# uc-vision/taichi_gaussian_rasterizer

Measured on AMD Instinct MI355X. Metric: Mpixels/s fwd+bwd @ 2048x2048, 1M Gaussians, higher is better.
Workload: dtype f32

## Files before the change

### taichi_gaussian_rasterizer_amd/csrc/frame.cpp

```cpp

#include <string.h>

#include "gs_common.h"

namespace {

int64_t a256(int64_t bytes) { return gs_align_up(bytes > 0 ? bytes : 1, 256); }

struct Dims {
  int64_t n, P, T;
  int C, F, col0, RS, tiles_x, tiles_y, local_h, D;
  bool want_vis;
};

int frame_dims(const GsFrame* f, Dims* d) {
  GS_REQUIRE(f != nullptr, GS_ERR_INVALID_ARGUMENT, "frame: descriptor is NULL");
  if (int rc = gs_check_cfg(&f->cfg)) return rc;
  GS_REQUIRE(f->n >= 0 && f->n < (int64_t(1) << 31), GS_ERR_INVALID_ARGUMENT, "frame: %lld gaussians", (long long)f->n);
  GS_REQUIRE(f->width > 0 && f->height > 0, GS_ERR_INVALID_ARGUMENT, "frame: image size %dx%d", f->width, f->height);
  GS_REQUIRE(f->sh_degree >= -1 && f->sh_degree <= 3, GS_ERR_UNSUPPORTED, "frame: SH degree %d", f->sh_degree);
  GS_REQUIRE(f->channels >= 1 && f->channels <= (f->sh_degree >= 0 ? GS_MAX_SH_CHANNELS : GS_MAX_FEATURES - 2),
             GS_ERR_UNSUPPORTED, "frame: %d feature channels", f->channels);
  const int ts = f->cfg.tile_size;
  GsShard sh;
// ... 23 lines not shown

template <typename T>
T* at(void* base, int64_t off) { return reinterpret_cast<T*>(static_cast<char*>(base) + off); }

struct StageTimer {
  void* const* events;
  int rc = GS_OK;
  void mark(int stage, int end, void* stream) {
    if (!events || !events[2 * stage + end]) return;
    if (hipEventRecord(static_cast<hipEvent_t>(events[2 * stage + end]), static_cast<hipStream_t>(stream)) != hipSuccess) {
      gs_set_error("frame: hipEventRecord of a stage timer failed");
      rc = GS_ERR_LAUNCH;
    }
  }
};

}

int gs_project_fwd_ex(int64_t n, const float* position, const float* log_scaling, const float* rotation,
                      const float* alpha_logit, const float* T_camera_world, const float* projection, int32_t width,
                      int32_t height, double near_plane, double far_plane, const GsRasterConfig* cfg, float* points,
                      float* depth, float* ndc_depth, int64_t* indexes, int32_t* slot_of, int32_t* num_visible,
                      float* depth_features, int32_t depth_features_stride, float* camera_pos, void* scratch,
                      int64_t scratch_bytes, float* zero_rows, int32_t zero_row_floats, const GsMapBinPlan* bin,
                      void* stream);

extern "C" int gs_frame_layout(const GsFrame* f, GsFrameLayout* out) {
  Dims d;
  if (int rc = frame_dims(f, &d)) return rc;
  GS_REQUIRE(out != nullptr, GS_ERR_INVALID_ARGUMENT, "gs_frame_layout: layout is NULL");
// ... 157 lines not shown
  if (lists) {
    int32_t* touched = at<int32_t>(workspace, L.touched);
    if ((rc = gs_map_touched_list(d.n, v_dev, d.T, stage, map_bytes, touched, counts + 1, indexes, d.n,
                                  f->exchange_world, at<int64_t>(workspace, L.owner_counts), f->exchange_rank,
                                  counts + 2, stream)))
      return rc;
    if (f->sh_degree >= 0) {
      tm.mark(GS_FWD_COLOURS, 0, stream);
      if ((rc = gs_sh_fwd_rows(d.n, touched, counts + 1, d.C, f->sh_degree, feature, position, indexes, cam_pos, colours,
                               d.F, stream)))
        return rc;
      tm.mark(GS_FWD_COLOURS, 1, stream);
    }
  }
  const int32_t tile_hint = f->max_tile_hint > 0 ? -f->max_tile_hint : 0;
  tm.mark(GS_FWD_MAP_FINISH, 0, stream);
  if ((rc = gs_map_finish(d.n, v_dev, f->k_capacity, tile_hint, points, ndc, f->width, f->height, cfg, f->use_depth16,
                          tile_ranges, o2p, nullptr, at<char>(scratch, L.s_pairs), shard, stage, map_bytes,
                          stream)))
    return rc;
  tm.mark(GS_FWD_MAP_FINISH, 1, stream);
  tm.mark(GS_FWD_RASTER, 0, stream);
  if ((rc = gs_raster_fwd_bg(d.n, d.F, points, feats, tile_ranges, o2p, f->k_capacity, f->width, f->height, &rcfg,
                             tile_order, counts + 7, image, alpha, vis, shard, background, d.col0, stream)))
    return rc;
  tm.mark(GS_FWD_RASTER, 1, stream);
  if (f->render_depth &&
      (rc = gs_depth_split_fwd(d.P, d.C, image, alpha, 1e-6f, at<float>(workspace, L.out_image),
                               at<float>(workspace, L.img_depth), at<float>(workspace, L.img_var), stream)))
    return rc;
  if (f->render_median_depth) {
    GsRasterConfig pick = f->cfg;
    pick.use_alpha_blending = 0;
    pick.saturate_threshold = 0.5f;
    pick.compute_visibility = 0;
    pick.compute_point_heuristic = 0;
    if ((rc = gs_raster_fwd(d.n, 1, points, depth, tile_ranges, o2p, f->k_capacity, f->width, f->height, &pick,
                            tile_order, counts + 7, at<float>(workspace, L.median),
                            at<float>(scratch, L.s_median_cover), nullptr, shard, stream)))
// ... 216 lines not shown
```

### taichi_gaussian_rasterizer_amd/csrc/gs_common.h

```cpp
#pragma once

#include <hip/hip_runtime.h>
#include <stdint.h>
#include <stdio.h>

#include "../../include/gsplat_hip.h"

#define GS_WAVE 64

void gs_set_error(const char* fmt, ...);

#define GS_REQUIRE(cond, status, ...)  \
  do {                                 \
    if (!(cond)) {                     \
      gs_set_error(__VA_ARGS__);       \
      return (status);                 \
    }                                  \
  } while (0)

#define GS_CHECK_LAUNCH(name)                                                   \
  do {                                                                          \
    hipError_t e_ = hipGetLastError();                                          \
    if (e_ != hipSuccess) {                                                     \
      gs_set_error("%s: launch failed: %s", name, hipGetErrorString(e_));       \
// ... 101 lines not shown
  const void* st_rows;
  const int* block_offsets;
  const int* block_counts;
  int num_blocks;
  float inv_far, ndc_denom;
  float* points; float* depth; float* ndc; int64_t* indexes; int* slot_of; int* num_visible;
  float* depth_feat; int depth_feat_stride;
  void* zero_rows; int zero_row_v4;
};
int gs_map_compact_bin(const GsMapBinPlan* plan, const GsCompactArgs* c, void* stream);
int gs_map_bin_counters(const GsMapBinPlan* plan, int64_t n, int32_t** words, int32_t* count);
int gs_map_prepare_ex(int64_t v, const int32_t* v_dev, const float* points, int32_t width, int32_t height,
                      const GsRasterConfig* cfg, int64_t k_capacity, int32_t* tile_ranges, int32_t* counts_out,
                      int32_t* counts_host, int32_t* tile_order, const GsRowShard* shard, void* scratch,
                      int64_t scratch_bytes, int binned, void* stream);
int gs_rows_add(int64_t v, int32_t row_floats, float* rows, const float* add_points, const float* add_depth,
                int32_t depth_col, void* stream);

#ifdef __HIPCC__

__device__ __forceinline__ int gs_xcd_remap(int block, int n) {
  const int chunk = (n + 7) >> 3;
  const int item = (block & 7) * chunk + (block >> 3);
  return ((block >> 3) < chunk && item < n) ? item : -1;
}

template <int CTRL, int ROW_MASK = 0xf, int BANK_MASK = 0xf>
__device__ __forceinline__ float gs_dpp_add(float x) {
  const int moved = __builtin_amdgcn_update_dpp(0, __float_as_int(x), CTRL, ROW_MASK, BANK_MASK, false);
  return x + __int_as_float(moved);
// ... 173 lines not shown
```

### taichi_gaussian_rasterizer_amd/csrc/mapper.hip

```cpp

#include "gs_common.h"
#include "../../include/gs_detmath.h"

namespace {

struct GridQuery {
  float ib00, ib01, ib10, ib11;
  float rel_min_x, rel_min_y;
  int min_tx, min_ty, span_x, span_y;
};

__device__ __forceinline__ GridQuery grid_query(const float* g, int Wp, int Hp, int tile_size, float alpha_thr) {
  GridQuery q;
  const float mx = g[0], my = g[1], ax = g[2], ay = g[3], sgx = g[4], sgy = g[5], alpha = g[6];
  if (!(alpha > alpha_thr)) {
    q.ib00 = q.ib01 = q.ib10 = q.ib11 = q.rel_min_x = q.rel_min_y = 0.f;
    q.min_tx = q.min_ty = q.span_x = q.span_y = 0;
    return q;
  }
  const float gscale = gs_det_sqrtf(2.0f * gs_det_logf(__fdiv_rn(alpha, alpha_thr)));
  const float sx = sgx * gscale, sy = sgy * gscale;
  const float a2x = -ay, a2y = ax;
  const float v1x = ax * sx, v1y = ay * sx, v2x = a2x * sy, v2y = a2y * sy;
  const float ex = gs_det_sqrtf(v1x * v1x + v2x * v2x), ey = gs_det_sqrtf(v1y * v1y + v2y * v2y);
// ... 47 lines not shown
  int depth16;
  GsShard sh;
};

__device__ __forceinline__ bool any_owned_row(const GsShard& sh, int lo, int hi) { return gs_shard_any_row(sh, lo, hi); }
__device__ __forceinline__ int local_tile(const MapArgs& a, int gx, int gy) {
  return gs_shard_local_row(a.sh, gy) * a.tiles_wide + gx;
}

__device__ __forceinline__ int64_t live_count(const MapArgs& a) {
  if (a.v_dev == nullptr) return a.v;
  const int64_t d = *a.v_dev;
  return d < a.v ? d : a.v;
}

__device__ __forceinline__ int wave_inclusive_scan(int x) {
  x += __builtin_amdgcn_update_dpp(0, x, 0x111, 0xf, 0xf, true);
  x += __builtin_amdgcn_update_dpp(0, x, 0x112, 0xf, 0xf, true);
  x += __builtin_amdgcn_update_dpp(0, x, 0x114, 0xf, 0xf, true);
  x += __builtin_amdgcn_update_dpp(0, x, 0x118, 0xf, 0xf, true);
  x += __builtin_amdgcn_update_dpp(0, x, 0x142, 0xa, 0xf, false);
  x += __builtin_amdgcn_update_dpp(0, x, 0x143, 0xc, 0xf, false);
  return x;
}

__device__ __forceinline__ int block_exclusive_scan(int x, int* s_wave, int& sum) {
  const int lane = threadIdx.x & 63, wv = threadIdx.x >> 6;
  const int inc = wave_inclusive_scan(x);
  if (lane == 63) s_wave[wv] = inc;
  __syncthreads();
  int before = 0;
  sum = 0;
#pragma unroll
  for (int w = 0; w < 16; ++w) {
    const int tot = s_wave[w];
    sum += tot;
    before += w < wv ? tot : 0;
  }
  __syncthreads();
// ... 523 lines not shown
    }
  }
  for (uint64_t todo = wide_lanes; todo != 0ull; todo &= todo - 1ull) {
    const int gi = __shfl(i, __ffsll(static_cast<unsigned long long>(todo)) - 1);
    const GridQuery w = grid_query(a.points + 7 * int64_t(gi), a.Wp, a.Hp, a.tile_size, a.thr);
    const uint64_t pair = (uint64_t(depth_key(a.depth[gi], a.depth16 != 0)) << 32) | uint64_t(uint32_t(gi));
    const int total = w.span_x * w.span_y;
    for (int k = lane; k < total; k += 64) {
      const int ty = k / w.span_x, tx = k - ty * w.span_x;
      if (gs_shard_owns(a.sh, ty + w.min_ty) && test_tile(w, tx, ty, a.tile_size))
        place(tx + w.min_tx, ty + w.min_ty, pair);
    }
  }
}

template <int THREADS>
__device__ __forceinline__ void bitonic_sort(uint64_t* data, int n, int t) {
  int np2 = 1;
  while (np2 < n) np2 <<= 1;
  for (int k = 2; k <= np2; k <<= 1) {
    for (int i = t; i < n; i += THREADS) {
      const int l = i ^ (k - 1);
      if (l > i && l < n) {
        const uint64_t x = data[i], y = data[l];
        if (x > y) { data[i] = y; data[l] = x; }
      }
    }
    __syncthreads();
    for (int j = k >> 2; j > 0; j >>= 1) {
      for (int i = t; i < n; i += THREADS) {
        const int l = i ^ j;
        if (l > i && l < n) {
          const uint64_t x = data[i], y = data[l];
          if (x > y) { data[i] = y; data[l] = x; }
        }
      }
      __syncthreads();
    }
  }
}

template <int THREADS, int CAP>
__device__ __forceinline__ uint64_t* lds_merge_sort(uint64_t* a, uint64_t* b, int n, int t) {
  const int np = (n + 255) & ~255;
  for (int i = n + t; i < np; i += THREADS) a[i] = 0xFFFFFFFF00000000ull | uint64_t(i);
  __syncthreads();
  const int lane = t & 63;
  for (int base = (t >> 6) * 256; base < np; base += (THREADS >> 6) * 256) {
    uint64_t* chunk = a + base;
    uint64_t mine[4];
    int rank[4];
#pragma unroll
    for (int q = 0; q < 4; ++q) { mine[q] = chunk[q * 64 + lane]; rank[q] = 0; }
    for (int j = 0; j < 64; ++j) {
#pragma unroll
// ... 96 lines not shown
      data = lds_merge_sort<THREADS, CAP>(s_a, s_b, n, t);
    } else {
      __syncthreads();
      bitonic_sort<THREADS>(stage, n, t);
      data = stage;
    }
    for (int i = t; i < n; i += THREADS) {
      const uint64_t kv = data[i];
      keys_out[lo + i] = K(uint32_t(kv >> 32) ^ bias);
      values_out[lo + i] = values[lo + int(uint32_t(kv))];
    }
    __syncthreads();
  }
}

template <int R>
__device__ __forceinline__ void rank_sort_rows(uint64_t* s_key, int n, int lane, int start, int tile, int* o2p,
                                               uint64_t* keys_out, int shift) {
  uint64_t mine[R];
  int rank[R];
#pragma unroll
  for (int q = 0; q < R; ++q) {
    mine[q] = s_key[q * 64 + lane];
    rank[q] = 0;
  }
  if (R == 1) {
    for (int j = 0; j < n; ++j) rank[0] += s_key[j] < mine[0] ? 1 : 0;
  } else {
    for (int j = 0; j < 64; ++j) {
#pragma unroll
      for (int q = 0; q < R; ++q) rank[q] += s_key[q * 64 + j] < mine[q] ? 1 : 0;
    }
#pragma unroll
    for (int q = 0; q < R; ++q) s_key[q * 64 + rank[q]] = mine[q];
    __syncthreads();
#pragma unroll
    for (int q = 0; q < R; ++q) {
#pragma unroll
      for (int p = 0; p < R; ++p) {
        if (p == q) continue;
        const uint64_t* row = s_key + p * 64;
        int pos = 0;
#pragma unroll
        for (int step = 32; step >= 1; step >>= 1) pos += row[pos + step - 1] < mine[q] ? step : 0;
        pos += row[pos] < mine[q] ? 1 : 0;
        rank[q] += pos;
      }
    }
  }
#pragma unroll
  for (int q = 0; q < R; ++q) {
    if ((mine[q] >> 32) != 0xFFFFFFFFull) {
      o2p[start + rank[q]] = int(uint32_t(mine[q]));
      if (keys_out) keys_out[start + rank[q]] = (mine[q] >> 32) | (uint64_t(uint32_t(tile)) << shift);
    }
  }
}

#ifndef GS_SORT_BINS
#define GS_SORT_BINS 1
#endif
constexpr int SORT_BINS = 256, BIN_LIMIT = 40;

template <int R>
__device__ __forceinline__ bool bucket_sort_rows(uint64_t* s_key, int* s_hist, int n, int lane, int start, int tile,
                                                 int* o2p, uint64_t* keys_out, int shift) {
  uint64_t mine[R];
  uint32_t mn = 0xFFFFFFFFu, mx = 0u;
#pragma unroll
  for (int q = 0; q < R; ++q) {
    mine[q] = s_key[q * 64 + lane];
    if (q * 64 + lane < n) {
      const uint32_t hi = uint32_t(mine[q] >> 32);
      mn = min(mn, hi);
      mx = max(mx, hi);
    }
  }
#pragma unroll
  for (int off = 32; off > 0; off >>= 1) {
    mn = min(mn, uint32_t(__shfl_xor(int(mn), off)));
    mx = max(mx, uint32_t(__shfl_xor(int(mx), off)));
  }
  const float scale = float(SORT_BINS) / (float(mx - mn) + 1.0f);
#pragma unroll
  for (int k = 0; k < SORT_BINS / 64; ++k) s_hist[k * 64 + lane] = 0;
  __syncthreads();
  int bin[R], arrival[R];
#pragma unroll
  for (int q = 0; q < R; ++q) {
    bin[q] = 0; arrival[q] = 0;
    if (q * 64 + lane < n) {
      bin[q] = min(SORT_BINS - 1, int(float(uint32_t(mine[q] >> 32) - mn) * scale));
      arrival[q] = atomicAdd(&s_hist[bin[q]], 1);
    }
  }
  __syncthreads();
  int c[SORT_BINS / 64], local = 0, fullest = 0;
#pragma unroll
  for (int k = 0; k < SORT_BINS / 64; ++k) {
    c[k] = s_hist[lane * (SORT_BINS / 64) + k];
    local += c[k];
    fullest = max(fullest, c[k]);
  }
#pragma unroll
  for (int off = 32; off > 0; off >>= 1) fullest = max(fullest, __shfl_xor(fullest, off));
  if (fullest > BIN_LIMIT) return false;
  int run = wave_inclusive_scan(local) - local;
  __syncthreads();
#pragma unroll
  for (int k = 0; k < SORT_BINS / 64; ++k) {
    s_hist[lane * (SORT_BINS / 64) + k] = run;
    run += c[k];
  }
  if (lane == 63) s_hist[SORT_BINS] = run;
  __syncthreads();
#pragma unroll
  for (int q = 0; q < R; ++q)
    if (q * 64 + lane < n) s_key[s_hist[bin[q]] + arrival[q]] = mine[q];
  __syncthreads();
#pragma unroll
  for (int q = 0; q < R; ++q) {
    if (q * 64 + lane >= n) continue;
    const int b0 = s_hist[bin[q]], b1 = s_hist[bin[q] + 1];
    int rank = b0;
    for (int j = b0; j < b1; ++j) rank += s_key[j] < mine[q] ? 1 : 0;
    o2p[start + rank] = int(uint32_t(mine[q]));
    if (keys_out) keys_out[start + rank] = (mine[q] >> 32) | (uint64_t(uint32_t(tile)) << shift);
  }
  return true;
}

template <int RMAX>
__global__ __launch_bounds__(64, 6) void tile_rank_sort_kernel(int num_tiles, const int2* tile_ranges,
                                                            uint64_t* pairs, int* o2p, uint64_t* keys_out,
                                                            int depth16, int skip_full) {
  __shared__ uint64_t s_key[64 * RMAX];
  __shared__ int s_hist[SORT_BINS + 1];
  const int tile = gs_xcd_remap(blockIdx.x, num_tiles);
  if (tile < 0) return;
  const int2 r = tile_ranges[tile];
  const int n = r.y - r.x;
  if (n <= 0) return;
  const int lane = threadIdx.x;
  const int shift = depth16 ? 16 : 32;
  if (n > 64 * RMAX) {
// ... 404 lines not shown
                       m.region_start, m.chunk_start, hist, m.qcache);
    GS_CHECK_LAUNCH("gs_map_prepare/count");
  }
  hipLaunchKernelGGL(map_scan_kernel, dim3(tile_order ? 2 : 1), dim3(1024), 0, s, num_tiles, hist,
                     reinterpret_cast<int2*>(tile_ranges), cursors, counts_out, k_capacity, tile_order, v_dev,
                     counts_host, v > 0 ? m.region_start + rg.num_regions : nullptr);
  GS_CHECK_LAUNCH("gs_map_prepare/scan");
  return GS_OK;
}

extern "C" int gs_map_finish(int64_t v, const int32_t* v_dev, int64_t k, int32_t max_tile_count, const float* points,
                             const float* depth, int32_t width, int32_t height, const GsRasterConfig* cfg,
                             int32_t use_depth16, const int32_t* tile_ranges, int32_t* overlap_to_point,
                             uint64_t* sorted_keys, void* pair_scratch, const GsRowShard* shard, void* scratch,
                             int64_t scratch_bytes, void* stream) {
  MapArgs a;
  if (int rc = fill_args(a, v, points, depth, width, height, cfg, use_depth16, shard)) return rc;
  a.v_dev = v_dev;
  if (k == 0 || v == 0) return GS_OK;
  const int num_tiles = a.tiles_wide * a.sh.local_rows;
  GS_REQUIRE(points && depth && tile_ranges && overlap_to_point && pair_scratch && scratch, GS_ERR_INVALID_ARGUMENT,
             "gs_map_finish: NULL buffer");
  GS_REQUIRE(scratch_bytes >= gs_map_scratch_bytes(v, num_tiles), GS_ERR_SCRATCH_TOO_SMALL,
             "gs_map_finish: scratch too small");
  hipStream_t s = static_cast<hipStream_t>(stream);
  const MapScratch m = carve(scratch, v, num_tiles);
  int* cursors = m.cursors;
  const RegionGrid rg = make_grid(a);
  uint64_t* pairs = static_cast<uint64_t*>(pair_scratch);
  hipLaunchKernelGGL(emit_binned_kernel, dim3(unsigned(gs_div_up(v, CHUNK)) + unsigned(rg.num_regions)), dim3(CHUNK),
                     size_t(rg.win) * rg.win * 8, s,
                     a, rg, m.order, m.region_start, m.chunk_start, cursors, pairs, m.qcache);
  GS_CHECK_LAUNCH("gs_map_finish/emit");
  const int grid = 8 * int(gs_div_up(num_tiles, 8));
  const int2* r = reinterpret_cast<const int2*>(tile_ranges);
  const bool exact = max_tile_count > 0;
  const int guess = exact ? max_tile_count : (max_tile_count < 0 ? -max_tile_count : 1024);
  const bool big_pass = guess > 512;
  const int skip_full = (exact || big_pass) ? 1 : 0;
  int covered;
  if (guess <= 256) {
    covered = 256;
    hipLaunchKernelGGL((tile_rank_sort_kernel<4>), dim3(grid), dim3(64), 0, s, num_tiles, r, pairs, overlap_to_point,
                       sorted_keys, use_depth16, skip_full);
  } else {
    covered = 512;
    hipLaunchKernelGGL((tile_rank_sort_kernel<8>), dim3(grid), dim3(64), 0, s, num_tiles, r, pairs, overlap_to_point,
                       sorted_keys, use_depth16, skip_full);
  }
  if (big_pass) {
    constexpr int SMALL = 1024, MID = 2048, CAP = 8192;
    const bool mid_pass = guess > SMALL, huge_pass = guess > MID;
// ... 133 lines not shown
```

### taichi_gaussian_rasterizer_amd/csrc/raster_fwd.hip

```cpp

#include "gs_common.h"
#include "raster_pdf.h"

namespace {

struct FwdArgs {
  const float* points;
  const float* features;
  const int2* ranges;
  const int* o2p;
  float* image;
  float* alpha;
  float* visibility;
  int W, H, F;
  int tiles_wide;
  int tile_size;
  int sub_x, sub_y;
  int num_items;
  int num_tiles;
  const int* heavy;
  int heavy_cap;
  const int* tile_order;
  float cmax, thr, inv_thr, sat_level;
  float cut;
  int blend, vis, aa;
  GsShard sh;
  const float* bg;
  int bg_off;
};

__device__ __forceinline__ void tile_origin(const FwdArgs& a, int tile, int& x0, int& y0, int& yout0) {
  const int lty = tile / a.tiles_wide;
  x0 = (tile - lty * a.tiles_wide) * a.tile_size;
  y0 = gs_shard_global_row(a.sh, lty) * a.tile_size;
  yout0 = lty * a.tile_size;
}

template <int NB, int FP, int MODE>
__device__ __forceinline__ void raster_fwd_body(const FwdArgs& a, int tile, int x0, int y0, int yout0,
                                                float4 (*s_geo)[(MODE == 2 ? 3 : 2) + (FP + 3) / 4], float* s_vis,
                                                int* s_idx) {
  constexpr int GEO_V4 = MODE == 2 ? 3 : 2, FEAT_V4 = (FP + 3) / 4;
  constexpr bool FULL = MODE == 2, VIS = MODE == 1 || MODE == 2, QUANT = MODE == 3;
  const bool blend = QUANT ? false : (FULL ? a.blend != 0 : true);
  const int lane = threadIdx.x;
  const int lx = lane & 7, ly = lane >> 3;
  float Xf[NB], Yf[NB], Tr[NB], acc[NB][FP];
  bool inb[NB], done[NB];
#pragma unroll
  for (int b = 0; b < NB; ++b) {
    const int X = x0 + (b & 1) * 8 + lx, Y = y0 + (b >> 1) * 8 + ly;
    inb[b] = X < a.W && Y < a.H;
    Xf[b] = FULL ? float(X) + 0.5f : float((b & 1) * 8 + lx) + 0.5f;
    Yf[b] = FULL ? float(Y) + 0.5f : float((b >> 1) * 8 + ly) + 0.5f;
    Tr[b] = inb[b] ? 1.0f : 0.0f;
    done[b] = false;
#pragma unroll
    for (int c = 0; c < FP; ++c) acc[b][c] = 0.0f;
  }

  const int2 range_v = a.ranges[tile];
  int2 range;
  range.x = __builtin_amdgcn_readfirstlane(range_v.x);
  range.y = __builtin_amdgcn_readfirstlane(range_v.y);
  const float k_exp = 0.84932180028801904f;

  for (int g0 = range.x; g0 < range.y; g0 += 64) {
    int live = 0;
    if (blend) {
#pragma unroll
      for (int b = 0; b < NB; ++b)
        if (__ballot(Tr[b] > a.cut) != 0ull) live |= 1 << b;
    } else {
#pragma unroll
      for (int b = 0; b < NB; ++b)
        if (__ballot(inb[b] && !done[b]) != 0ull) live |= 1 << b;
    }
    if (live == 0) break;
    const int cnt = __builtin_amdgcn_readfirstlane(min(64, range.y - g0));
    int staged_mask = 0;
    if (lane < cnt) {
      const int idx = a.o2p[g0 + lane];
      const float* p = a.points + int64_t(idx) * 7;
      const float mx = p[0], my = p[1], ax = p[2], ay = p[3], sx = p[4], sy = p[5], al = p[6];
      const float isx = gs_rcp_fast(sx), isy = gs_rcp_fast(sy);
      const float Ax = ax * isx * k_exp, Ay = ay * isx * k_exp;
      const float Bx = -ay * isy * k_exp, By = ax * isy * k_exp;
      int mask = 0;
      if (FULL && a.aa) {
        mask = gs_sub_block_mask_antialias<NB>(ax, ay, sx, sy, al, a.inv_thr, s_sig(0.5f, isx) - s_sig(-0.5f, isx),
                                               s_sig(0.5f, isy) - s_sig(-0.5f, isy), float(x0) + 0.5f - mx,
                                               float(y0) + 0.5f - my);
      } else if (al > a.thr) {
        mask = gs_sub_block_mask<NB>(Ax, Ay, Bx, By, __log2f(al * a.inv_thr), float(x0) + 0.5f - mx,
                                     float(y0) + 0.5f - my);
      }
      staged_mask = mask;
// ... 115 lines not shown
    const int X = x0 + (b & 1) * 8 + lx, Y = y0 + (b >> 1) * 8 + ly;
    const int64_t pix = int64_t(Y - y0 + yout0) * a.W + X;
    float* out = a.image + pix * a.F;
    if (a.bg != nullptr) {
#pragma unroll
      for (int c = 0; c < FP; ++c)
        if (c >= a.bg_off && c < a.F) acc[b][c] = __builtin_fmaf(Tr[b], a.bg[c - a.bg_off], acc[b][c]);
    }
#pragma unroll
    for (int c = 0; c < FP; ++c)
      if (c < a.F) out[c] = acc[b][c];
    a.alpha[pix] = blend ? 1.0f - Tr[b] : (Tr[b] < 1.0f ? 1.0f : 0.0f);
  }
}

template <int NB, int FP, int MODE>
__global__ __launch_bounds__(64) void raster_fwd_kernel(const FwdArgs a) {
  __shared__ float4 s_geo[64][(MODE == 2 ? 3 : 2) + (FP + 3) / 4];
  __shared__ float s_vis[(MODE == 1 || MODE == 2) ? 64 : 1];
  __shared__ int s_idx[(MODE == 1 || MODE == 2) ? 64 : 1];
  const int per_tile = a.sub_x * a.sub_y;
  constexpr int RW = NB == 1 ? 8 : 16, RH = NB == 4 ? 16 : 8;
  int tile, quad;
  if (a.tile_order) {
    const int b = blockIdx.x;
    const int heavy = (NB > 1 && a.heavy) ? min(*a.heavy, a.heavy_cap) : 0;
    if (NB > 1 && b < 4 * heavy) {
      tile = a.tile_order[b >> 2];
      int x0, y0, yout0;
      tile_origin(a, tile, x0, y0, yout0);
      x0 += (b & 1) * 8; y0 += ((b >> 1) & 1) * 8; yout0 += ((b >> 1) & 1) * 8;
      if (x0 < a.W && y0 < a.H) raster_fwd_body<1, FP, MODE>(a, tile, x0, y0, yout0, s_geo, s_vis, s_idx);
      return;
    }
    const int c = b - 4 * heavy, rank = heavy + c / per_tile;
    if (rank >= a.num_tiles) return;
    tile = a.tile_order[rank];
    quad = c % per_tile;
  } else {
    const int item = gs_xcd_remap(blockIdx.x, a.num_items);
    if (item < 0) return;
    tile = item / per_tile;
    quad = item - tile * per_tile;
  }
  int x0, y0, yout0;
  tile_origin(a, tile, x0, y0, yout0);
  x0 += (quad % a.sub_x) * RW; y0 += (quad / a.sub_x) * RH; yout0 += (quad / a.sub_x) * RH;
  if (x0 >= a.W || y0 >= a.H) return;
  raster_fwd_body<NB, FP, MODE>(a, tile, x0, y0, yout0, s_geo, s_vis, s_idx);
}

template <int NB, int MODE>
int launch_fp(const FwdArgs& a, hipStream_t s) {
  const int grid = 8 * int(gs_div_up(a.num_items + (a.heavy ? 4 * a.heavy_cap : 0), 8));
  if (MODE == 3 && a.F == 1) hipLaunchKernelGGL((raster_fwd_kernel<NB, 1, MODE>), dim3(grid), dim3(64), 0, s, a);
  else if (a.F <= 3) hipLaunchKernelGGL((raster_fwd_kernel<NB, 3, MODE>), dim3(grid), dim3(64), 0, s, a);
  else if (a.F <= 5) hipLaunchKernelGGL((raster_fwd_kernel<NB, 5, MODE>), dim3(grid), dim3(64), 0, s, a);
  else if (a.F <= 8) hipLaunchKernelGGL((raster_fwd_kernel<NB, 8, MODE>), dim3(grid), dim3(64), 0, s, a);
  else hipLaunchKernelGGL((raster_fwd_kernel<NB, 32, MODE>), dim3(grid), dim3(64), 0, s, a);
  GS_CHECK_LAUNCH("gs_raster_fwd");
  return GS_OK;
}

}

extern "C" int gs_raster_fwd_bg(int64_t v, int32_t num_features, const float* points, const float* features,
                                const int32_t* tile_ranges, const int32_t* overlap_to_point, int64_t k, int32_t width,
                                int32_t height, const GsRasterConfig* cfg, const int32_t* tile_order,
                                const int32_t* heavy_tiles, float* image, float* alpha, float* visibility,
                                const GsRowShard* shard, const float* background, int32_t background_offset,
                                void* stream) {
  if (int rc = gs_check_cfg(cfg)) return rc;
  if (int rc = gs_check_background("gs_raster_fwd", cfg->use_alpha_blending, background != nullptr, background_offset,
                                   num_features))
    return rc;
  GS_REQUIRE(width > 0 && height > 0, GS_ERR_INVALID_ARGUMENT, "gs_raster_fwd: image size %dx%d", width, height);
  GS_REQUIRE(num_features >= 1 && num_features <= GS_MAX_FEATURES, GS_ERR_UNSUPPORTED,
             "gs_raster_fwd: feature width %d not in [1,%d]", num_features, GS_MAX_FEATURES);
  GS_REQUIRE(image && alpha && tile_ranges, GS_ERR_INVALID_ARGUMENT, "gs_raster_fwd: NULL output or ranges");
  GS_REQUIRE(k == 0 || (points && features && overlap_to_point), GS_ERR_INVALID_ARGUMENT,
             "gs_raster_fwd: NULL input with %lld overlaps", (long long)k);
  const bool vis = cfg->compute_visibility || cfg->compute_point_heuristic;
  GS_REQUIRE(!vis || visibility || v == 0, GS_ERR_INVALID_ARGUMENT, "gs_raster_fwd: visibility buffer is NULL");
  const int ts = cfg->tile_size;
  FwdArgs a;
  a.points = points; a.features = features; a.ranges = reinterpret_cast<const int2*>(tile_ranges);
  a.o2p = overlap_to_point; a.image = image; a.alpha = alpha; a.visibility = visibility;
  a.W = width; a.H = height; a.F = num_features;
  a.tiles_wide = int(gs_div_up(width, ts));
  a.tile_size = ts;
  if (int rc = gs_make_shard(shard, int(gs_div_up(height, ts)), &a.sh)) return rc;
  const int num_tiles = a.tiles_wide * a.sh.local_rows;
  if (num_tiles == 0) return GS_OK;
  const int nb = gs_raster_sub_blocks(cfg, num_tiles, 0);
  a.sub_x = ts / (nb == 1 ? 8 : 16);
  a.sub_y = ts / (nb == 4 ? 16 : 8);
  a.num_items = num_tiles * a.sub_x * a.sub_y;
  a.tile_order = tile_order;
  a.num_tiles = num_tiles;
  a.heavy = (tile_order && ts == 16 && nb > 1) ? heavy_tiles : nullptr;
  a.heavy_cap = num_tiles / 4;
  if (cfg->tune_no_heavy_split) a.heavy = nullptr;
  a.cmax = cfg->clamp_max_alpha; a.thr = cfg->alpha_threshold; a.inv_thr = 1.0f / cfg->alpha_threshold;
  a.sat_level = 1.0f - cfg->saturate_threshold;
  a.cut = cfg->forward_cut > 2.98023223876953125e-08f ? cfg->forward_cut : 2.98023223876953125e-08f;
  a.blend = cfg->use_alpha_blending; a.vis = vis; a.aa = cfg->antialias;
  a.bg = background; a.bg_off = background ? background_offset : 0;
  hipStream_t s = static_cast<hipStream_t>(stream);
  const int mode = (!a.blend && !a.aa && !a.vis) ? 3 : (!a.blend || a.aa) ? 2 : a.vis ? 1 : 0;
// ... 19 lines not shown
```

### taichi_gaussian_rasterizer_amd/fused.py

```python
from __future__ import annotations

import ctypes
import weakref

import torch

from . import _native as nv
from .data_types import RasterConfig
from .spherical_harmonics import check_sh_degree

_K_HINT = {}
FRAME_CALLS = True
_PINNED = {}


def _pinned_counts(dev: torch.device) -> torch.Tensor:
    ring = _PINNED.get(dev.index)
    if ring is None:
        ring = _PINNED[dev.index] = dict(bufs=[torch.empty((8,), dtype=torch.int32).pin_memory() for _ in range(4)],
                                         at=0)
    ring["at"] = (ring["at"] + 1) % len(ring["bufs"])
    return ring["bufs"][ring["at"]]


# ... 381 lines not shown
    def backward(ctx, *grads):
        return _FrameRender.backward(ctx, *grads)[:5] + (None,) * (len(ctx.needs_input_grad) - 5)


def fused_supported(gaussians, camera_params, use_sh: bool, render_median_depth: bool) -> bool:
    f = gaussians.feature
    if gaussians.position.shape[0] == 0 or not f.is_cuda or f.dtype != torch.float32:
        return False
    if use_sh:
        return f.ndim == 3 and f.shape[1] <= 8
    return f.ndim == 2 and 1 <= f.shape[1] <= 30


def _capacity(hint):
    k_cap = -(-(int(hint[0] * 1.25) + 4096) // 65536) * 65536
    tile_hint = next((c for c in (256, 512, 1024, 2048) if hint[1] <= c), 4096)
    return k_cap, tile_hint


def render_fused(gaussians, camera_params, config: RasterConfig, render_depth: bool, use_depth16: bool,
                 shard=None, group=None, render_median_depth: bool = False, exchange: str = "dense",
                 grad_mode: str = "replicated", owned=None, owned_range=None, sparse_grad: bool = False,
                 background=None, differentiable_weight: bool = False):
    import weakref

    from .renderer import Rendering
    if shard is not None and (background is not None or differentiable_weight):
        raise NotImplementedError("render_fused: a sharded frame has neither a background nor a differentiable "
                                  "image_weight (parallel.render_gaussians_sharded does not take the arguments)")
    holder = {}
    args = (gaussians.position.contiguous(), gaussians.log_scaling.contiguous(), gaussians.rotation.contiguous(),
# ... 40 lines not shown
```

Baseline: 3977.

## Defer per-tile depth sort into the forward raster kernel behind env flag

Adds an optional path where the map-finish stage skips its per-tile sort and the forward raster kernel sorts each tile's key segment in LDS (bucket or rank sort), then reads gaussian indices from shared memory. The sorted order is still written to overlap_to_point for the backward pass. The path is gated by the GS_SORT_IN_RASTER environment variable, so it is off by default. Separately, it adds waves-per-EU occupancy hints to the raster kernel and a 384 tile-hint bucket in the Python capacity helper; both of those apply unconditionally.

```diff
diff --git a/taichi_gaussian_rasterizer_amd/csrc/frame.cpp b/taichi_gaussian_rasterizer_amd/csrc/frame.cpp
--- a/taichi_gaussian_rasterizer_amd/csrc/frame.cpp
+++ b/taichi_gaussian_rasterizer_amd/csrc/frame.cpp
@@ -1,4 +1,5 @@
 
+#include <stdlib.h>
 #include <string.h>
 
 #include "gs_common.h"
@@ -61,6 +62,14 @@
     }
   }
 };
+
+int sort_in_raster_enabled() {
+  static const int on = [] {
+    const char* e = getenv("GS_SORT_IN_RASTER");
+    return (e != nullptr && e[0] == '1' && e[1] == '\0') ? 1 : 0;
+  }();
+  return on;
+}
 
 }
 
@@ -248,15 +257,17 @@
     }
   }
   const int32_t tile_hint = f->max_tile_hint > 0 ? -f->max_tile_hint : 0;
+  int32_t sort_deferred = 0;
   tm.mark(GS_FWD_MAP_FINISH, 0, stream);
-  if ((rc = gs_map_finish(d.n, v_dev, f->k_capacity, tile_hint, points, ndc, f->width, f->height, cfg, f->use_depth16,
-                          tile_ranges, o2p, nullptr, at<char>(scratch, L.s_pairs), shard, stage, map_bytes,
-                          stream)))
+  if ((rc = gs_map_finish_ex(d.n, v_dev, f->k_capacity, tile_hint, points, ndc, f->width, f->height, cfg,
+                             f->use_depth16, tile_ranges, o2p, nullptr, at<char>(scratch, L.s_pairs), shard, stage,
+                             map_bytes, sort_in_raster_enabled(), &sort_deferred, stream)))
     return rc;
   tm.mark(GS_FWD_MAP_FINISH, 1, stream);
   tm.mark(GS_FWD_RASTER, 0, stream);
-  if ((rc = gs_raster_fwd_bg(d.n, d.F, points, feats, tile_ranges, o2p, f->k_capacity, f->width, f->height, &rcfg,
-                             tile_order, counts + 7, image, alpha, vis, shard, background, d.col0, stream)))
+  if ((rc = gs_raster_fwd_ex(d.n, d.F, points, feats, tile_ranges, o2p, f->k_capacity, f->width, f->height, &rcfg,
+                             tile_order, counts + 7, image, alpha, vis, shard, background, d.col0,
+                             sort_deferred ? at<uint64_t>(scratch, L.s_pairs) : nullptr, stream)))
     return rc;
   tm.mark(GS_FWD_RASTER, 1, stream);
   if (f->render_depth &&
diff --git a/taichi_gaussian_rasterizer_amd/csrc/gs_common.h b/taichi_gaussian_rasterizer_amd/csrc/gs_common.h
--- a/taichi_gaussian_rasterizer_amd/csrc/gs_common.h
+++ b/taichi_gaussian_rasterizer_amd/csrc/gs_common.h
@@ -139,6 +139,17 @@
                       const GsRasterConfig* cfg, int64_t k_capacity, int32_t* tile_ranges, int32_t* counts_out,
                       int32_t* counts_host, int32_t* tile_order, const GsRowShard* shard, void* scratch,
                       int64_t scratch_bytes, int binned, void* stream);
+#define GS_RASTER_SORT_MAX 384
+int gs_map_finish_ex(int64_t v, const int32_t* v_dev, int64_t k, int32_t max_tile_count, const float* points,
+                     const float* depth, int32_t width, int32_t height, const GsRasterConfig* cfg, int32_t use_depth16,
+                     const int32_t* tile_ranges, int32_t* overlap_to_point, uint64_t* sorted_keys, void* pair_scratch,
+                     const GsRowShard* shard, void* scratch, int64_t scratch_bytes, int32_t sort_in_raster,
+                     int32_t* sort_deferred, void* stream);
+int gs_raster_fwd_ex(int64_t v, int32_t num_features, const float* points, const float* features,
+                     const int32_t* tile_ranges, int32_t* overlap_to_point, int64_t k, int32_t width, int32_t height,
+                     const GsRasterConfig* cfg, const int32_t* tile_order, const int32_t* heavy_tiles, float* image,
+                     float* alpha, float* visibility, const GsRowShard* shard, const float* background,
+                     int32_t background_offset, uint64_t* pairs, void* stream);
 int gs_rows_add(int64_t v, int32_t row_floats, float* rows, const float* add_points, const float* add_depth,
                 int32_t depth_col, void* stream);
 
diff --git a/taichi_gaussian_rasterizer_amd/csrc/mapper.hip b/taichi_gaussian_rasterizer_amd/csrc/mapper.hip
--- a/taichi_gaussian_rasterizer_amd/csrc/mapper.hip
+++ b/taichi_gaussian_rasterizer_amd/csrc/mapper.hip
@@ -1,6 +1,7 @@
 
 #include "gs_common.h"
 #include "../../include/gs_detmath.h"
+#include "tile_sort.h"
 
 namespace {
 
@@ -85,15 +86,6 @@
   return d < a.v ? d : a.v;
 }
 
-__device__ __forceinline__ int wave_inclusive_scan(int x) {
-  x += __builtin_amdgcn_update_dpp(0, x, 0x111, 0xf, 0xf, true);
-  x += __builtin_amdgcn_update_dpp(0, x, 0x112, 0xf, 0xf, true);
-  x += __builtin_amdgcn_update_dpp(0, x, 0x114, 0xf, 0xf, true);
-  x += __builtin_amdgcn_update_dpp(0, x, 0x118, 0xf, 0xf, true);
-  x += __builtin_amdgcn_update_dpp(0, x, 0x142, 0xa, 0xf, false);
-  x += __builtin_amdgcn_update_dpp(0, x, 0x143, 0xc, 0xf, false);
-  return x;
-}
 
 __device__ __forceinline__ int block_exclusive_scan(int x, int* s_wave, int& sum) {
   const int lane = threadIdx.x & 63, wv = threadIdx.x >> 6;
@@ -647,31 +639,6 @@
   }
 }
 
-template <int THREADS>
-__device__ __forceinline__ void bitonic_sort(uint64_t* data, int n, int t) {
-  int np2 = 1;
-  while (np2 < n) np2 <<= 1;
-  for (int k = 2; k <= np2; k <<= 1) {
-    for (int i = t; i < n; i += THREADS) {
-      const int l = i ^ (k - 1);
-      if (l > i && l < n) {
-        const uint64_t x = data[i], y = data[l];
-        if (x > y) { data[i] = y; data[l] = x; }
-      }
-    }
-    __syncthreads();
-    for (int j = k >> 2; j > 0; j >>= 1) {
-      for (int i = t; i < n; i += THREADS) {
-        const int l = i ^ j;
-        if (l > i && l < n) {
-          const uint64_t x = data[i], y = data[l];
-          if (x > y) { data[i] = y; data[l] = x; }
-        }
-      }
-      __syncthreads();
-    }
-  }
-}
 
 template <int THREADS, int CAP>
 __device__ __forceinline__ uint64_t* lds_merge_sort(uint64_t* a, uint64_t* b, int n, int t) {
@@ -798,121 +765,6 @@
   }
 }
 
-template <int R>
-__device__ __forceinline__ void rank_sort_rows(uint64_t* s_key, int n, int lane, int start, int tile, int* o2p,
-                                               uint64_t* keys_out, int shift) {
-  uint64_t mine[R];
-  int rank[R];
-#pragma unroll
-  for (int q = 0; q < R; ++q) {
-    mine[q] = s_key[q * 64 + lane];
-    rank[q] = 0;
-  }
-  if (R == 1) {
-    for (int j = 0; j < n; ++j) rank[0] += s_key[j] < mine[0] ? 1 : 0;
-  } else {
-    for (int j = 0; j < 64; ++j) {
-#pragma unroll
-      for (int q = 0; q < R; ++q) rank[q] += s_key[q * 64 + j] < mine[q] ? 1 : 0;
-    }
-#pragma unroll
-    for (int q = 0; q < R; ++q) s_key[q * 64 + rank[q]] = mine[q];
-    __syncthreads();
-#pragma unroll
-    for (int q = 0; q < R; ++q) {
-#pragma unroll
-      for (int p = 0; p < R; ++p) {
-        if (p == q) continue;
-        const uint64_t* row = s_key + p * 64;
-        int pos = 0;
-#pragma unroll
-        for (int step = 32; step >= 1; step >>= 1) pos += row[pos + step - 1] < mine[q] ? step : 0;
-        pos += row[pos] < mine[q] ? 1 : 0;
-        rank[q] += pos;
-      }
-    }
-  }
-#pragma unroll
-  for (int q = 0; q < R; ++q) {
-    if ((mine[q] >> 32) != 0xFFFFFFFFull) {
-      o2p[start + rank[q]] = int(uint32_t(mine[q]));
-      if (keys_out) keys_out[start + rank[q]] = (mine[q] >> 32) | (uint64_t(uint32_t(tile)) << shift);
-    }
-  }
-}
-
-#ifndef GS_SORT_BINS
-#define GS_SORT_BINS 1
-#endif
-constexpr int SORT_BINS = 256, BIN_LIMIT = 40;
-
-template <int R>
-__device__ __forceinline__ bool bucket_sort_rows(uint64_t* s_key, int* s_hist, int n, int lane, int start, int tile,
-                                                 int* o2p, uint64_t* keys_out, int shift) {
-  uint64_t mine[R];
-  uint32_t mn = 0xFFFFFFFFu, mx = 0u;
-#pragma unroll
-  for (int q = 0; q < R; ++q) {
-    mine[q] = s_key[q * 64 + lane];
-    if (q * 64 + lane < n) {
-      const uint32_t hi = uint32_t(mine[q] >> 32);
-      mn = min(mn, hi);
-      mx = max(mx, hi);
-    }
-  }
-#pragma unroll
-  for (int off = 32; off > 0; off >>= 1) {
-    mn = min(mn, uint32_t(__shfl_xor(int(mn), off)));
-    mx = max(mx, uint32_t(__shfl_xor(int(mx), off)));
-  }
-  const float scale = float(SORT_BINS) / (float(mx - mn) + 1.0f);
-#pragma unroll
-  for (int k = 0; k < SORT_BINS / 64; ++k) s_hist[k * 64 + lane] = 0;
-  __syncthreads();
-  int bin[R], arrival[R];
-#pragma unroll
-  for (int q = 0; q < R; ++q) {
-    bin[q] = 0; arrival[q] = 0;
-    if (q * 64 + lane < n) {
-      bin[q] = min(SORT_BINS - 1, int(float(uint32_t(mine[q] >> 32) - mn) * scale));
-      arrival[q] = atomicAdd(&s_hist[bin[q]], 1);
-    }
-  }
-  __syncthreads();
-  int c[SORT_BINS / 64], local = 0, fullest = 0;
-#pragma unroll
-  for (int k = 0; k < SORT_BINS / 64; ++k) {
-    c[k] = s_hist[lane * (SORT_BINS / 64) + k];
-    local += c[k];
-    fullest = max(fullest, c[k]);
-  }
-#pragma unroll
-  for (int off = 32; off > 0; off >>= 1) fullest = max(fullest, __shfl_xor(fullest, off));
-  if (fullest > BIN_LIMIT) return false;
-  int run = wave_inclusive_scan(local) - local;
-  __syncthreads();
-#pragma unroll
-  for (int k = 0; k < SORT_BINS / 64; ++k) {
-    s_hist[lane * (SORT_BINS / 64) + k] = run;
-    run += c[k];
-  }
-  if (lane == 63) s_hist[SORT_BINS] = run;
-  __syncthreads();
-#pragma unroll
-  for (int q = 0; q < R; ++q)
-    if (q * 64 + lane < n) s_key[s_hist[bin[q]] + arrival[q]] = mine[q];
-  __syncthreads();
-#pragma unroll
-  for (int q = 0; q < R; ++q) {
-    if (q * 64 + lane >= n) continue;
-    const int b0 = s_hist[bin[q]], b1 = s_hist[bin[q] + 1];
-    int rank = b0;
-    for (int j = b0; j < b1; ++j) rank += s_key[j] < mine[q] ? 1 : 0;
-    o2p[start + rank] = int(uint32_t(mine[q]));
-    if (keys_out) keys_out[start + rank] = (mine[q] >> 32) | (uint64_t(uint32_t(tile)) << shift);
-  }
-  return true;
-}
 
 template <int RMAX>
 __global__ __launch_bounds__(64, 6) void tile_rank_sort_kernel(int num_tiles, const int2* tile_ranges,
@@ -1347,6 +1199,16 @@
                              int32_t use_depth16, const int32_t* tile_ranges, int32_t* overlap_to_point,
                              uint64_t* sorted_keys, void* pair_scratch, const GsRowShard* shard, void* scratch,
                              int64_t scratch_bytes, void* stream) {
+  return gs_map_finish_ex(v, v_dev, k, max_tile_count, points, depth, width, height, cfg, use_depth16, tile_ranges,
+                          overlap_to_point, sorted_keys, pair_scratch, shard, scratch, scratch_bytes, 0, nullptr, stream);
+}
+
+int gs_map_finish_ex(int64_t v, const int32_t* v_dev, int64_t k, int32_t max_tile_count, const float* points,
+                     const float* depth, int32_t width, int32_t height, const GsRasterConfig* cfg, int32_t use_depth16,
+                     const int32_t* tile_ranges, int32_t* overlap_to_point, uint64_t* sorted_keys, void* pair_scratch,
+                     const GsRowShard* shard, void* scratch, int64_t scratch_bytes, int32_t sort_in_raster,
+                     int32_t* sort_deferred, void* stream) {
+  if (sort_deferred) *sort_deferred = 0;
   MapArgs a;
   if (int rc = fill_args(a, v, points, depth, width, height, cfg, use_depth16, shard)) return rc;
   a.v_dev = v_dev;
@@ -1369,6 +1231,11 @@
   const int2* r = reinterpret_cast<const int2*>(tile_ranges);
   const bool exact = max_tile_count > 0;
   const int guess = exact ? max_tile_count : (max_tile_count < 0 ? -max_tile_count : 1024);
+  if (sort_in_raster && sort_deferred && !exact && guess <= GS_RASTER_SORT_MAX && cfg->tile_size == 16 &&
+      sorted_keys == nullptr && gs_raster_sub_blocks(cfg, num_tiles, 0) == 4) {
+    *sort_deferred = 1;
+    return GS_OK;
+  }
   const bool big_pass = guess > 512;
   const int skip_full = (exact || big_pass) ? 1 : 0;
   int covered;
diff --git a/taichi_gaussian_rasterizer_amd/csrc/raster_fwd.hip b/taichi_gaussian_rasterizer_amd/csrc/raster_fwd.hip
--- a/taichi_gaussian_rasterizer_amd/csrc/raster_fwd.hip
+++ b/taichi_gaussian_rasterizer_amd/csrc/raster_fwd.hip
@@ -1,6 +1,7 @@
 
 #include "gs_common.h"
 #include "raster_pdf.h"
+#include "tile_sort.h"
 
 namespace {
 
@@ -27,7 +28,37 @@
   GsShard sh;
   const float* bg;
   int bg_off;
+  uint64_t* pairs;
+  int* o2p_out;
 };
+
+constexpr int SORT_MAX = GS_RASTER_SORT_MAX;
+
+__device__ __forceinline__ void sort_bucket_in_wave(uint64_t* s_key, int* s_aux, const uint64_t* seg, int n, int lane,
+                                                    int start, int* o2p) {
+  const int rows = (n + 63) >> 6;
+  for (int i = lane; i < rows * 64; i += 64) s_key[i] = i < n ? seg[i] : (0xFFFFFFFF00000000ull | uint64_t(i));
+  __syncthreads();
+  if (GS_SORT_BINS && rows >= 2) {
+    bool done = false;
+    switch (rows) {
+      case 2: done = bucket_sort_rows<2, true>(s_key, s_aux, n, lane, start, 0, o2p, nullptr, 0, s_aux); break;
+      case 3: done = bucket_sort_rows<3, true>(s_key, s_aux, n, lane, start, 0, o2p, nullptr, 0, s_aux); break;
+      case 4: done = bucket_sort_rows<4, true>(s_key, s_aux, n, lane, start, 0, o2p, nullptr, 0, s_aux); break;
+      case 5: done = bucket_sort_rows<5, true>(s_key, s_aux, n, lane, start, 0, o2p, nullptr, 0, s_aux); break;
+      default: done = bucket_sort_rows<6, true>(s_key, s_aux, n, lane, start, 0, o2p, nullptr, 0, s_aux); break;
+    }
+    if (done) return;
+  }
+  switch (rows) {
+    case 1: rank_sort_rows<1, true>(s_key, n, lane, start, 0, o2p, nullptr, 0, s_aux); break;
+    case 2: rank_sort_rows<2, true>(s_key, n, lane, start, 0, o2p, nullptr, 0, s_aux); break;
+    case 3: rank_sort_rows<3, true>(s_key, n, lane, start, 0, o2p, nullptr, 0, s_aux); break;
+    case 4: rank_sort_rows<4, true>(s_key, n, lane, start, 0, o2p, nullptr, 0, s_aux); break;
+    case 5: rank_sort_rows<5, true>(s_key, n, lane, start, 0, o2p, nullptr, 0, s_aux); break;
+    default: rank_sort_rows<6, true>(s_key, n, lane, start, 0, o2p, nullptr, 0, s_aux); break;
+  }
+}
 
 __device__ __forceinline__ void tile_origin(const FwdArgs& a, int tile, int& x0, int& y0, int& yout0) {
   const int lty = tile / a.tiles_wide;
@@ -36,14 +67,32 @@
   yout0 = lty * a.tile_size;
 }
 
-template <int NB, int FP, int MODE>
+template <int NB, int FP, int MODE, bool SORT>
 __device__ __forceinline__ void raster_fwd_body(const FwdArgs& a, int tile, int x0, int y0, int yout0,
                                                 float4 (*s_geo)[(MODE == 2 ? 3 : 2) + (FP + 3) / 4], float* s_vis,
-                                                int* s_idx) {
+                                                int* s_idx, int* s_aux, bool publish) {
   constexpr int GEO_V4 = MODE == 2 ? 3 : 2, FEAT_V4 = (FP + 3) / 4;
   constexpr bool FULL = MODE == 2, VIS = MODE == 1 || MODE == 2, QUANT = MODE == 3;
   const bool blend = QUANT ? false : (FULL ? a.blend != 0 : true);
   const int lane = threadIdx.x;
+  const int2 range_v = a.ranges[tile];
+  int2 range;
+  range.x = __builtin_amdgcn_readfirstlane(range_v.x);
+  range.y = __builtin_amdgcn_readfirstlane(range_v.y);
+  bool lds_idx = false;
+  if (SORT && a.pairs != nullptr && range.y > range.x) {
+    const int n = range.y - range.x;
+    if (n <= SORT_MAX) {
+      sort_bucket_in_wave(reinterpret_cast<uint64_t*>(&s_geo[0][0]), s_aux, a.pairs + range.x, n, lane, range.x,
+                          publish ? a.o2p_out : nullptr);
+      lds_idx = true;
+    } else {
+      uint64_t* gseg = a.pairs + range.x;
+      bitonic_sort<64>(gseg, n, lane);
+      for (int i = lane; i < n; i += 64) a.o2p_out[range.x + i] = int(uint32_t(gseg[i]));
+    }
+    __syncthreads();
+  }
   const int lx = lane & 7, ly = lane >> 3;
   float Xf[NB], Yf[NB], Tr[NB], acc[NB][FP];
   bool inb[NB], done[NB];
@@ -59,10 +108,6 @@
     for (int c = 0; c < FP; ++c) acc[b][c] = 0.0f;
   }
 
-  const int2 range_v = a.ranges[tile];
-  int2 range;
-  range.x = __builtin_amdgcn_readfirstlane(range_v.x);
-  range.y = __builtin_amdgcn_readfirstlane(range_v.y);
   const float k_exp = 0.84932180028801904f;
 
   for (int g0 = range.x; g0 < range.y; g0 += 64) {
@@ -80,7 +125,7 @@
     const int cnt = __builtin_amdgcn_readfirstlane(min(64, range.y - g0));
     int staged_mask = 0;
     if (lane < cnt) {
-      const int idx = a.o2p[g0 + lane];
+      const int idx = (SORT && lds_idx) ? s_aux[g0 - range.x + lane] : a.o2p[g0 + lane];
       const float* p = a.points + int64_t(idx) * 7;
       const float mx = p[0], my = p[1], ax = p[2], ay = p[3], sx = p[4], sy = p[5], al = p[6];
       const float isx = gs_rcp_fast(sx), isy = gs_rcp_fast(sy);
@@ -226,29 +271,52 @@
   }
 }
 
+constexpr int fwd_min_waves(int nb, int fp, int mode) {
+  if (nb != 4) return 1;
+  if (mode == 2) return fp <= 3 ? 6 : fp <= 5 ? 5 : fp <= 8 ? 4 : 1;
+  return fp <= 3 ? 8 : fp <= 5 ? 7 : fp <= 8 ? 5 : 2;
+}
+
 template <int NB, int FP, int MODE>
-__global__ __launch_bounds__(64) void raster_fwd_kernel(const FwdArgs a) {
+__global__ __launch_bounds__(64) __attribute__((amdgpu_waves_per_eu(fwd_min_waves(NB, FP, MODE))))
+void raster_fwd_kernel(const FwdArgs a) {
   __shared__ float4 s_geo[64][(MODE == 2 ? 3 : 2) + (FP + 3) / 4];
   __shared__ float s_vis[(MODE == 1 || MODE == 2) ? 64 : 1];
   __shared__ int s_idx[(MODE == 1 || MODE == 2) ? 64 : 1];
+  constexpr bool SORT = NB == 4;
+  __shared__ int s_aux[SORT ? SORT_MAX : 1];
+  static_assert(SORT_MAX * 8 <= int(sizeof(s_geo)) && SORT_MAX >= SORT_BINS + 1, "the sort's arena and bin table");
   const int per_tile = a.sub_x * a.sub_y;
   constexpr int RW = NB == 1 ? 8 : 16, RH = NB == 4 ? 16 : 8;
   int tile, quad;
   if (a.tile_order) {
     const int b = blockIdx.x;
     const int heavy = (NB > 1 && a.heavy) ? min(*a.heavy, a.heavy_cap) : 0;
-    if (NB > 1 && b < 4 * heavy) {
+    bool split = NB > 1 && b < 4 * heavy;
+    if (split) {
       tile = a.tile_order[b >> 2];
+      if (SORT && a.pairs != nullptr) {
+        const int2 r = a.ranges[tile];
+        if (r.y - r.x > SORT_MAX) {
+          if ((b & 3) != 0) return;
+          split = false;
+          quad = 0;
+        }
+      }
+    } else {
+      const int c = b - 4 * heavy, rank = heavy + c / per_tile;
+      if (rank >= a.num_tiles) return;
+      tile = a.tile_order[rank];
+      quad = c % per_tile;
+    }
+    if (split) {
       int x0, y0, yout0;
       tile_origin(a, tile, x0, y0, yout0);
       x0 += (b & 1) * 8; y0 += ((b >> 1) & 1) * 8; yout0 += ((b >> 1) & 1) * 8;
-      if (x0 < a.W && y0 < a.H) raster_fwd_body<1, FP, MODE>(a, tile, x0, y0, yout0, s_geo, s_vis, s_idx);
+      if (x0 < a.W && y0 < a.H)
+        raster_fwd_body<1, FP, MODE, SORT>(a, tile, x0, y0, yout0, s_geo, s_vis, s_idx, s_aux, (b & 3) == 0);
       return;
     }
-    const int c = b - 4 * heavy, rank = heavy + c / per_tile;
-    if (rank >= a.num_tiles) return;
-    tile = a.tile_order[rank];
-    quad = c % per_tile;
   } else {
     const int item = gs_xcd_remap(blockIdx.x, a.num_items);
     if (item < 0) return;
@@ -259,7 +327,7 @@
   tile_origin(a, tile, x0, y0, yout0);
   x0 += (quad % a.sub_x) * RW; y0 += (quad / a.sub_x) * RH; yout0 += (quad / a.sub_x) * RH;
   if (x0 >= a.W || y0 >= a.H) return;
-  raster_fwd_body<NB, FP, MODE>(a, tile, x0, y0, yout0, s_geo, s_vis, s_idx);
+  raster_fwd_body<NB, FP, MODE, SORT>(a, tile, x0, y0, yout0, s_geo, s_vis, s_idx, s_aux, true);
 }
 
 template <int NB, int MODE>
@@ -282,6 +350,16 @@
                                 const int32_t* heavy_tiles, float* image, float* alpha, float* visibility,
                                 const GsRowShard* shard, const float* background, int32_t background_offset,
                                 void* stream) {
+  return gs_raster_fwd_ex(v, num_features, points, features, tile_ranges, const_cast<int32_t*>(overlap_to_point), k,
+                          width, height, cfg, tile_order, heavy_tiles, image, alpha, visibility, shard, background,
+                          background_offset, nullptr, stream);
+}
+
+int gs_raster_fwd_ex(int64_t v, int32_t num_features, const float* points, const float* features,
+                     const int32_t* tile_ranges, int32_t* overlap_to_point, int64_t k, int32_t width, int32_t height,
+                     const GsRasterConfig* cfg, const int32_t* tile_order, const int32_t* heavy_tiles, float* image,
+                     float* alpha, float* visibility, const GsRowShard* shard, const float* background,
+                     int32_t background_offset, uint64_t* pairs, void* stream) {
   if (int rc = gs_check_cfg(cfg)) return rc;
   if (int rc = gs_check_background("gs_raster_fwd", cfg->use_alpha_blending, background != nullptr, background_offset,
                                    num_features))
@@ -305,6 +383,10 @@
   const int num_tiles = a.tiles_wide * a.sh.local_rows;
   if (num_tiles == 0) return GS_OK;
   const int nb = gs_raster_sub_blocks(cfg, num_tiles, 0);
+  GS_REQUIRE(pairs == nullptr || (ts == 16 && nb == 4), GS_ERR_UNSUPPORTED,
+             "gs_raster_fwd: the in-wave sort needs 16-pixel tiles and whole-tile waves (tile size %d, %d sub-blocks)",
+             ts, nb);
+  a.pairs = k > 0 ? pairs : nullptr; a.o2p_out = overlap_to_point;
   a.sub_x = ts / (nb == 1 ? 8 : 16);
   a.sub_y = ts / (nb == 4 ? 16 : 8);
   a.num_items = num_tiles * a.sub_x * a.sub_y;
diff --git a/taichi_gaussian_rasterizer_amd/csrc/tile_sort.h b/taichi_gaussian_rasterizer_amd/csrc/tile_sort.h
--- /dev/null
+++ b/taichi_gaussian_rasterizer_amd/csrc/tile_sort.h
@@ -0,0 +1,181 @@
+#pragma once
+
+#include "gs_common.h"
+
+namespace {
+
+__device__ __forceinline__ int wave_inclusive_scan(int x) {
+  x += __builtin_amdgcn_update_dpp(0, x, 0x111, 0xf, 0xf, true);
+  x += __builtin_amdgcn_update_dpp(0, x, 0x112, 0xf, 0xf, true);
+  x += __builtin_amdgcn_update_dpp(0, x, 0x114, 0xf, 0xf, true);
+  x += __builtin_amdgcn_update_dpp(0, x, 0x118, 0xf, 0xf, true);
+  x += __builtin_amdgcn_update_dpp(0, x, 0x142, 0xa, 0xf, false);
+  x += __builtin_amdgcn_update_dpp(0, x, 0x143, 0xc, 0xf, false);
+  return x;
+}
+
+template <int THREADS>
+__device__ __forceinline__ void bitonic_sort(uint64_t* data, int n, int t) {
+  int np2 = 1;
+  while (np2 < n) np2 <<= 1;
+  for (int k = 2; k <= np2; k <<= 1) {
+    for (int i = t; i < n; i += THREADS) {
+      const int l = i ^ (k - 1);
+      if (l > i && l < n) {
+        const uint64_t x = data[i], y = data[l];
+        if (x > y) { data[i] = y; data[l] = x; }
+      }
+    }
+    __syncthreads();
+    for (int j = k >> 2; j > 0; j >>= 1) {
+      for (int i = t; i < n; i += THREADS) {
+        const int l = i ^ j;
+        if (l > i && l < n) {
+          const uint64_t x = data[i], y = data[l];
+          if (x > y) { data[i] = y; data[l] = x; }
+        }
+      }
+      __syncthreads();
+    }
+  }
+}
+
+template <int R, bool LDS_OUT = false>
+__device__ __forceinline__ void rank_sort_rows(uint64_t* s_key, int n, int lane, int start, int tile, int* o2p,
+                                               uint64_t* keys_out, int shift, int* s_out = nullptr) {
+  uint64_t mine[R];
+  int rank[R];
+#pragma unroll
+  for (int q = 0; q < R; ++q) {
+    mine[q] = s_key[q * 64 + lane];
+    rank[q] = 0;
+  }
+  if (R == 1) {
+    for (int j = 0; j < n; ++j) rank[0] += s_key[j] < mine[0] ? 1 : 0;
+  } else {
+    for (int j = 0; j < 64; ++j) {
+#pragma unroll
+      for (int q = 0; q < R; ++q) rank[q] += s_key[q * 64 + j] < mine[q] ? 1 : 0;
+      if (LDS_OUT) __builtin_amdgcn_sched_barrier(0);
+    }
+#pragma unroll
+    for (int q = 0; q < R; ++q) s_key[q * 64 + rank[q]] = mine[q];
+    __syncthreads();
+#pragma unroll
+    for (int q = 0; q < R; ++q) {
+#pragma unroll
+      for (int p = 0; p < R; ++p) {
+        if (p == q) continue;
+        const uint64_t* row = s_key + p * 64;
+        int pos = 0;
+#pragma unroll
+        for (int step = 32; step >= 1; step >>= 1) pos += row[pos + step - 1] < mine[q] ? step : 0;
+        pos += row[pos] < mine[q] ? 1 : 0;
+        rank[q] += pos;
+        if (LDS_OUT) {
+          asm volatile("" : "+v"(rank[q]));
+          __builtin_amdgcn_sched_barrier(0);
+        }
+      }
+    }
+  }
+#pragma unroll
+  for (int q = 0; q < R; ++q) {
+    if ((mine[q] >> 32) != 0xFFFFFFFFull) {
+      if (LDS_OUT) {
+        s_out[rank[q]] = int(uint32_t(mine[q]));
+        if (o2p) o2p[start + rank[q]] = int(uint32_t(mine[q]));
+        continue;
+      }
+      o2p[start + rank[q]] = int(uint32_t(mine[q]));
+      if (keys_out) keys_out[start + rank[q]] = (mine[q] >> 32) | (uint64_t(uint32_t(tile)) << shift);
+    }
+  }
+}
+
+#ifndef GS_SORT_BINS
+#define GS_SORT_BINS 1
+#endif
+constexpr int SORT_BINS = 256, BIN_LIMIT = 40;
+
+template <int R, bool LDS_OUT = false>
+__device__ __forceinline__ bool bucket_sort_rows(uint64_t* s_key, int* s_hist, int n, int lane, int start, int tile,
+                                                 int* o2p, uint64_t* keys_out, int shift, int* s_out = nullptr) {
+#pragma clang fp contract(off)
+  uint64_t mine[R];
+  uint32_t mn = 0xFFFFFFFFu, mx = 0u;
+#pragma unroll
+  for (int q = 0; q < R; ++q) {
+    mine[q] = s_key[q * 64 + lane];
+    if (q * 64 + lane < n) {
+      const uint32_t hi = uint32_t(mine[q] >> 32);
+      mn = min(mn, hi);
+      mx = max(mx, hi);
+    }
+  }
+#pragma unroll
+  for (int off = 32; off > 0; off >>= 1) {
+    mn = min(mn, uint32_t(__shfl_xor(int(mn), off)));
+    mx = max(mx, uint32_t(__shfl_xor(int(mx), off)));
+  }
+  const float scale = float(SORT_BINS) / (float(mx - mn) + 1.0f);
+#pragma unroll
+  for (int k = 0; k < SORT_BINS / 64; ++k) s_hist[k * 64 + lane] = 0;
+  __syncthreads();
+  int bin[R], arrival[R];
+#pragma unroll
+  for (int q = 0; q < R; ++q) {
+    bin[q] = 0; arrival[q] = 0;
+    if (q * 64 + lane < n) {
+      bin[q] = min(SORT_BINS - 1, int(float(uint32_t(mine[q] >> 32) - mn) * scale));
+      arrival[q] = atomicAdd(&s_hist[bin[q]], 1);
+    }
+  }
+  __syncthreads();
+  int c[SORT_BINS / 64], local = 0, fullest = 0;
+#pragma unroll
+  for (int k = 0; k < SORT_BINS / 64; ++k) {
+    c[k] = s_hist[lane * (SORT_BINS / 64) + k];
+    local += c[k];
+    fullest = max(fullest, c[k]);
+  }
+#pragma unroll
+  for (int off = 32; off > 0; off >>= 1) fullest = max(fullest, __shfl_xor(fullest, off));
+  if (fullest > BIN_LIMIT) return false;
+  int run = wave_inclusive_scan(local) - local;
+  __syncthreads();
+#pragma unroll
+  for (int k = 0; k < SORT_BINS / 64; ++k) {
+    s_hist[lane * (SORT_BINS / 64) + k] = run;
+    run += c[k];
+  }
+  if (lane == 63) s_hist[SORT_BINS] = run;
+  __syncthreads();
+#pragma unroll
+  for (int q = 0; q < R; ++q)
+    if (q * 64 + lane < n) s_key[s_hist[bin[q]] + arrival[q]] = mine[q];
+  __syncthreads();
+#pragma unroll
+  for (int q = 0; q < R; ++q) {
+    if (q * 64 + lane >= n) continue;
+    const int b0 = s_hist[bin[q]], b1 = s_hist[bin[q] + 1];
+    int rank = b0;
+    for (int j = b0; j < b1; ++j) rank += s_key[j] < mine[q] ? 1 : 0;
+    if (LDS_OUT) {
+      bin[q] = rank;
+      if (o2p) o2p[start + rank] = int(uint32_t(mine[q]));
+      continue;
+    }
+    o2p[start + rank] = int(uint32_t(mine[q]));
+    if (keys_out) keys_out[start + rank] = (mine[q] >> 32) | (uint64_t(uint32_t(tile)) << shift);
+  }
+  if (LDS_OUT) {
+    __syncthreads();
+#pragma unroll
+    for (int q = 0; q < R; ++q)
+      if (q * 64 + lane < n) s_out[bin[q]] = int(uint32_t(mine[q]));
+  }
+  return true;
+}
+
+}
diff --git a/taichi_gaussian_rasterizer_amd/fused.py b/taichi_gaussian_rasterizer_amd/fused.py
--- a/taichi_gaussian_rasterizer_amd/fused.py
+++ b/taichi_gaussian_rasterizer_amd/fused.py
@@ -419,7 +419,7 @@
 
 def _capacity(hint):
     k_cap = -(-(int(hint[0] * 1.25) + 4096) // 65536) * 65536
-    tile_hint = next((c for c in (256, 512, 1024, 2048) if hint[1] <= c), 4096)
+    tile_hint = next((c for c in (256, 384, 512, 1024, 2048) if hint[1] <= c), 4096)
     return k_cap, tile_hint
 
 
```

Result: slower. 3920 (-1.4%).
